# DocF/multispectral-object-detection

Hardware: AMD Instinct MI355X
Metric: image-pairs/sec fwd, yolov5l+CFTx3 640×640 bs64, 1/2/4/8 GPU (higher is better)
Workload: dtype bf16; 1 GPU; cfg3 (yolov5l_fusion_transformerx3_FLIR_aligned) two-stream forward, 640x640, 64 pairs/GPU, BN folded, pre-NMS detections; pairs_per_gpu=64, image_size=640, parallelism=batch-shard x1, hip_graph=True, two_hip_streams=False, forwards_in_flight=3, streams_per_forward_in_flight=1, single_in_flight_streams=2

## Files before the change

multispectral-object-detection_amd/csrc/focus_common.h:

```cpp
#pragma once
#include "cft_common.h"

template <typename IN>
__device__ __forceinline__ void load_pair(const IN* p, float scale, float& a, float& b);
template <>
__device__ __forceinline__ void load_pair<float>(const float* p, float scale, float& a, float& b) {
  const float2 t = *reinterpret_cast<const float2*>(p);
  a = t.x * scale;
  b = t.y * scale;
}
template <>
__device__ __forceinline__ void load_pair<f16_t>(const f16_t* p, float scale, float& a, float& b) {
  const f32x2_t t = __builtin_convertvector(*reinterpret_cast<const f16x2_t*>(p), f32x2_t);
  a = t[0] * scale;
  b = t[1] * scale;
}
template <>
__device__ __forceinline__ void load_pair<unsigned char>(const unsigned char* p, float scale, float& a, float& b) {
  const unsigned short t = *reinterpret_cast<const unsigned short*>(p);
  a = (float)(t & 0xffu) * scale;
  b = (float)(t >> 8) * scale;
}
```

multispectral-object-detection_amd/csrc/focus_conv.hip:

```cpp
#include "cft_common.h"
#include "focus_common.h"

struct FocusConvParams {
  const unsigned char* in;
  long sb, sc, sh;
  float scale;
  const unsigned char* w;
  const float* bias;
  unsigned char* y;
  int kpad, ldy, yoff;
  int Ho, Wo, tiles_x, bands;
};

template <typename T, typename IN, int NT, int ACT>
__global__ void __launch_bounds__(512) focus_conv_kernel(const FocusConvParams p) {
  constexpr int N = NT * 16, TW = 64, TH = 4, PW = TW + 2, PH = TH + 2;
  constexpr int W_BYTES = 3 * N * 128;
  constexpr int ZERO_OFF = PH * PW * 32;
  constexpr int SLD = N + 4;
  constexpr int VPR = N / 8;
  extern __shared__ __attribute__((aligned(16))) unsigned char smem[];
  unsigned char* sW = smem;
  unsigned char* sZ = smem + W_BYTES;

  const int tid = threadIdx.x, lane = tid & 63;
  const int wave = __builtin_amdgcn_readfirstlane(tid >> 6);
  const int lrow = lane & 15, lgrp = lane >> 4;
  const int b = blockIdx.x / p.bands, band = blockIdx.x - b * p.bands;
  const int y0 = band * TH;

  for (int idx = tid; idx < 3 * N * 8; idx += 512) {
    const int kt = idx / (N * 8);
    const int r = idx - kt * (N * 8);
    const int n = r >> 3, s = r & 7, g = s ^ (n & 7);
    *reinterpret_cast<gran_t*>(sW + kt * (N * 128) + n * 128 + (s << 4)) =
        *reinterpret_cast<const gran_t*>(p.w + ((long)n * p.kpad + kt * 64 + g * 8) * 2);
  }
  float bias_v[NT];
#pragma unroll
  for (int j = 0; j < NT; ++j) bias_v[j] = p.bias != nullptr ? p.bias[j * 16 + lrow] : 0.0f;
  float* stage = reinterpret_cast<float*>(sZ) + wave * (16 * SLD);
  const IN* img = reinterpret_cast<const IN*>(p.in) + (long)b * p.sb;
  const int wrow = wave >> 1, wx = (wave & 1) * 32;
  const int y = y0 + wrow;

  const bool owner = tid < PH * PW;
  const int py = tid / PW, px = tid - py * PW;
  const int zy = y0 - 1 + py;
  float raw[12];
#define FOCUS_FETCH(tx_)                                                                            \
  {                                                                                                 \
    const int zx = (tx_) * TW - 1 + px;                                                             \
    _Pragma("unroll") for (int e = 0; e < 12; ++e) raw[e] = 0.0f;                                   \
    if (owner && (unsigned)zy < (unsigned)p.Ho && (unsigned)zx < (unsigned)p.Wo) {                  \
      _Pragma("unroll") for (int c = 0; c < 3; ++c) {                                               \
        const IN* base = img + (long)c * p.sc + (long)(2 * zy) * p.sh + 2 * zx;                     \
        load_pair<IN>(base, p.scale, raw[0 + c], raw[6 + c]);         \
        load_pair<IN>(base + p.sh, p.scale, raw[3 + c], raw[9 + c]);  \
      }                                                                                             \
    }                                                                                               \
  }
  FOCUS_FETCH(0)

  for (int tx = 0; tx < p.tiles_x; ++tx) {
    const int x0 = tx * TW;
    if (owner) {
      float v[16];
#pragma unroll
      for (int e = 0; e < 12; ++e) v[e] = raw[e];
      v[12] = v[13] = v[14] = v[15] = 0.0f;
      gran_t* o = reinterpret_cast<gran_t*>(sZ + tid * 32);
      o[0] = Elem<T>::pack(v);
      o[1] = Elem<T>::pack(v + 8);
    }
    if (tid == PH * PW) *reinterpret_cast<gran_t*>(sZ + ZERO_OFF) = gran_t{0u, 0u, 0u, 0u};
    lds_barrier();
    if (tx + 1 < p.tiles_x) FOCUS_FETCH(tx + 1)

    f32x4_t acc[2][NT];
#pragma unroll
    for (int i = 0; i < 2; ++i)
#pragma unroll
      for (int j = 0; j < NT; ++j) acc[i][j] = f32x4_t{0.f, 0.f, 0.f, 0.f};
#pragma unroll
    for (int ks = 0; ks < 5; ++ks) {
      const int tap = ks * 2 + (lgrp >> 1), half = lgrp & 1;
      const int kh = tap / 3, kw = tap - kh * 3;
      const int abase = tap < 9 ? ((wrow + kh) * PW + wx + lrow + kw) * 32 + half * 16 : ZERO_OFF;
      const int astep = tap < 9 ? 16 * 32 : 0;
      gran_t af[2], bf[NT];
#pragma unroll
      for (int i = 0; i < 2; ++i) af[i] = *reinterpret_cast<const gran_t*>(sZ + abase + i * astep);
      const int kg = (ks & 1) * 4 + lgrp;
#pragma unroll
      for (int j = 0; j < NT; ++j) {
        const int n = j * 16 + lrow;
        bf[j] = *reinterpret_cast<const gran_t*>(sW + (ks >> 1) * (N * 128) + n * 128 + ((kg ^ (n & 7)) << 4));
      }
#pragma unroll
      for (int i = 0; i < 2; ++i)
#pragma unroll
        for (int j = 0; j < NT; ++j) acc[i][j] = mma_granule<T>(af[i], bf[j], acc[i][j]);
    }
    lds_barrier();

#pragma unroll
    for (int i = 0; i < 2; ++i) {
#pragma unroll
      for (int j = 0; j < NT; ++j)
#pragma unroll
        for (int e = 0; e < 4; ++e)
          stage[(lgrp * 4 + e) * SLD + j * 16 + lrow] = apply_act<ACT>(acc[i][j][e] + bias_v[j]);
      __builtin_amdgcn_fence(__ATOMIC_RELEASE, "wavefront");
      __builtin_amdgcn_wave_barrier();
      __builtin_amdgcn_fence(__ATOMIC_ACQUIRE, "wavefront");
      for (int it = lane; it < 16 * VPR; it += 64) {
        const int row = it / VPR, col = (it - row * VPR) * 8;
        const int x = x0 + wx + i * 16 + row;
        if (x < p.Wo && y < p.Ho) {
          const f32x4_t s0 = *reinterpret_cast<const f32x4_t*>(stage + row * SLD + col);
          const f32x4_t s1 = *reinterpret_cast<const f32x4_t*>(stage + row * SLD + col + 4);
          const float v[8] = {s0[0], s0[1], s0[2], s0[3], s1[0], s1[1], s1[2], s1[3]};
          const long m = ((long)b * p.Ho + y) * p.Wo + x;
          *reinterpret_cast<gran_t*>(p.y + (m * p.ldy + p.yoff + col) * 2) = Elem<T>::pack(v);
        }
      }
      __builtin_amdgcn_fence(__ATOMIC_RELEASE, "wavefront");
      __builtin_amdgcn_wave_barrier();
      __builtin_amdgcn_fence(__ATOMIC_ACQUIRE, "wavefront");
    }
    lds_barrier();
  }
#undef FOCUS_FETCH
}

template <typename T, typename IN, int NT, int ACT>
static int launch_focus_conv(const FocusConvParams& p, int B, hipStream_t stream) {
  constexpr int N = NT * 16;
  constexpr int patch = 6 * 66 * 32 + 16, strips = 8 * 16 * (N + 4) * 4;
  constexpr int smem_bytes = 3 * N * 128 + (patch > strips ? patch : strips);
  cft_allow_lds<&focus_conv_kernel<T, IN, NT, ACT>>(smem_bytes);
  hipLaunchKernelGGL((focus_conv_kernel<T, IN, NT, ACT>), dim3(B * p.bands), dim3(512), smem_bytes, stream, p);
  return cft_check_launch("focus_conv_kernel");
}

template <typename T, typename IN, int ACT>
static int dispatch_focus_conv(const FocusConvParams& p, int B, int n, hipStream_t stream) {
  switch (n) {
    case 32: return launch_focus_conv<T, IN, 2, ACT>(p, B, stream);
    case 48: return launch_focus_conv<T, IN, 3, ACT>(p, B, stream);
    case 64: return launch_focus_conv<T, IN, 4, ACT>(p, B, stream);
    default: return launch_focus_conv<T, IN, 5, ACT>(p, B, stream);
  }
}
template <typename T, typename IN>
static int dispatch_focus_act(const FocusConvParams& p, int B, int n, int act, hipStream_t stream) {
  return act == CFT_ACT_SILU ? dispatch_focus_conv<T, IN, CFT_ACT_SILU>(p, B, n, stream) : dispatch_focus_conv<T, IN, CFT_ACT_NONE>(p, B, n, stream);
}
template <typename T>
static int dispatch_focus_in(const FocusConvParams& p, int B, int n, int act, int in_kind, hipStream_t stream) {
  if (in_kind == 1) return dispatch_focus_act<T, unsigned char>(p, B, n, act, stream);
  if constexpr (sizeof(T) == 2 && !__is_same(T, uint16_t)) {
    if (in_kind == 2) return dispatch_focus_act<T, f16_t>(p, B, n, act, stream);
  }
  return dispatch_focus_act<T, float>(p, B, n, act, stream);
}

extern "C" int cft_focus_conv(const void* in, int in_kind, long stride_b, long stride_c, long stride_h, float scale,
                              const void* w, int kpad, const float* bias, void* y, int ldy, int yoff,
                              int B, int H, int W, int n, int act, int dtype, void* stream) {
  CFT_REQUIRE(in && w && y, "cft_focus_conv: null pointer");
  CFT_REQUIRE(dtype == CFT_BF16 || dtype == CFT_F16, "cft_focus_conv: dtype must be CFT_BF16 or CFT_F16");
  CFT_REQUIRE(in_kind >= 0 && in_kind <= 2, "cft_focus_conv: in_kind must be 0 (float), 1 (uint8) or 2 (half)");
  CFT_REQUIRE(in_kind != 2 || dtype == CFT_F16, "cft_focus_conv: half images require dtype CFT_F16");
  CFT_REQUIRE(B > 0 && H > 0 && W > 0 && (H % 2 == 0) && (W % 2 == 0), "cft_focus_conv: H and W must be even");
  CFT_REQUIRE(n == 32 || n == 48 || n == 64 || n == 80, "cft_focus_conv: n must be 32, 48, 64 or 80 (use cft_focus_s2d + cft_conv2d otherwise)");
  CFT_REQUIRE(kpad == 192, "cft_focus_conv: weights must be packed as [n][192] (3x3 taps x 16 channels, zero padded)");
  CFT_REQUIRE(act == CFT_ACT_SILU || act == CFT_ACT_NONE, "cft_focus_conv: activation must be SiLU or none");
  CFT_REQUIRE(ldy % 8 == 0 && yoff % 8 == 0 && ldy >= yoff + n, "cft_focus_conv: bad output ld/offset");
  CFT_REQUIRE(stride_h >= W && stride_c > 0 && stride_b > 0, "cft_focus_conv: bad strides");
  const long es = in_kind == 1 ? 1 : (in_kind == 2 ? 2 : 4);
  CFT_REQUIRE(((long)(size_t)in * 1 % (2 * es) == 0) && stride_h % 2 == 0 && stride_c % 2 == 0 && stride_b % 2 == 0,
              "cft_focus_conv: image rows must start on pixel-pair boundaries (pointer and strides even)");
  FocusConvParams p;
  p.in = (const unsigned char*)in; p.sb = stride_b; p.sc = stride_c; p.sh = stride_h; p.scale = scale;
  p.w = (const unsigned char*)w; p.bias = bias; p.y = (unsigned char*)y;
  p.kpad = kpad; p.ldy = ldy; p.yoff = yoff;
  p.Ho = H / 2; p.Wo = W / 2; p.tiles_x = (p.Wo + 63) / 64; p.bands = (p.Ho + 3) / 4;
  CFT_REQUIRE((long)B * p.bands < (1L << 31) && (long)B * p.Ho * p.Wo * ldy < (1L << 40), "cft_focus_conv: tensor too large");
  hipStream_t s = as_stream(stream);
  return dtype == CFT_BF16 ? dispatch_focus_in<uint16_t>(p, B, n, act, in_kind, s) : dispatch_focus_in<f16_t>(p, B, n, act, in_kind, s);
}
```

Baseline: 3689 image-pairs/sec.

## Separate focus-conv staging LDS from patch to overlap next-tile build with epilogue

When LDS allows, the focus conv kernel now gives the output staging strips their own region, separate from the input patch. This lets the next tile's patch be built and its global fetch issued right after the MMA loop, overlapping the epilogue stores and removing one barrier per tile. Raw image bits are now held undecoded in registers and converted only at build time, which cuts live registers. Weight loads are batched before the LDS stores. In exchange LDS use per block goes up, which may lower occupancy, and the control flow is more complex.

```diff
diff --git a/multispectral-object-detection_amd/csrc/focus_common.h b/multispectral-object-detection_amd/csrc/focus_common.h
--- a/multispectral-object-detection_amd/csrc/focus_common.h
+++ b/multispectral-object-detection_amd/csrc/focus_common.h
@@ -2,22 +2,40 @@
 #include "cft_common.h"
 
 template <typename IN>
-__device__ __forceinline__ void load_pair(const IN* p, float scale, float& a, float& b);
+struct ImagePair;
 template <>
-__device__ __forceinline__ void load_pair<float>(const float* p, float scale, float& a, float& b) {
-  const float2 t = *reinterpret_cast<const float2*>(p);
-  a = t.x * scale;
-  b = t.y * scale;
+struct ImagePair<float> {
+  typedef float2 bits;
+  static __device__ __forceinline__ bits zero() { return float2{0.0f, 0.0f}; }
+  static __device__ __forceinline__ bits load(const float* p) { return *reinterpret_cast<const float2*>(p); }
+  static __device__ __forceinline__ void convert(bits t, float scale, float& a, float& b) {
+    a = t.x * scale;
+    b = t.y * scale;
+  }
+};
+template <>
+struct ImagePair<f16_t> {
+  typedef f16x2_t bits;
+  static __device__ __forceinline__ bits zero() { return f16x2_t{(f16_t)0.0f, (f16_t)0.0f}; }
+  static __device__ __forceinline__ bits load(const f16_t* p) { return *reinterpret_cast<const f16x2_t*>(p); }
+  static __device__ __forceinline__ void convert(bits h, float scale, float& a, float& b) {
+    const f32x2_t t = __builtin_convertvector(h, f32x2_t);
+    a = t[0] * scale;
+    b = t[1] * scale;
+  }
+};
+template <>
+struct ImagePair<unsigned char> {
+  typedef unsigned short bits;
+  static __device__ __forceinline__ bits zero() { return 0; }
+  static __device__ __forceinline__ bits load(const unsigned char* p) { return *reinterpret_cast<const unsigned short*>(p); }
+  static __device__ __forceinline__ void convert(bits t, float scale, float& a, float& b) {
+    a = (float)(t & 0xffu) * scale;
+    b = (float)(t >> 8) * scale;
+  }
+};
+
+template <typename IN>
+__device__ __forceinline__ void load_pair(const IN* p, float scale, float& a, float& b) {
+  ImagePair<IN>::convert(ImagePair<IN>::load(p), scale, a, b);
 }
-template <>
-__device__ __forceinline__ void load_pair<f16_t>(const f16_t* p, float scale, float& a, float& b) {
-  const f32x2_t t = __builtin_convertvector(*reinterpret_cast<const f16x2_t*>(p), f32x2_t);
-  a = t[0] * scale;
-  b = t[1] * scale;
-}
-template <>
-__device__ __forceinline__ void load_pair<unsigned char>(const unsigned char* p, float scale, float& a, float& b) {
-  const unsigned short t = *reinterpret_cast<const unsigned short*>(p);
-  a = (float)(t & 0xffu) * scale;
-  b = (float)(t >> 8) * scale;
-}
diff --git a/multispectral-object-detection_amd/csrc/focus_conv.hip b/multispectral-object-detection_amd/csrc/focus_conv.hip
--- a/multispectral-object-detection_amd/csrc/focus_conv.hip
+++ b/multispectral-object-detection_amd/csrc/focus_conv.hip
@@ -12,6 +12,13 @@
   int Ho, Wo, tiles_x, bands;
 };
 
+template <int N>
+struct focus_lds {
+  static constexpr int weights = 3 * N * 128, patch = 6 * 66 * 32 + 16, strips = 8 * 16 * (N + 4) * 4;
+  static constexpr bool separate = weights + patch + strips <= 80 * 1024;
+  static constexpr int bytes = weights + (separate ? patch + strips : (patch > strips ? patch : strips));
+};
+
 template <typename T, typename IN, int NT, int ACT>
 __global__ void __launch_bounds__(512) focus_conv_kernel(const FocusConvParams p) {
   constexpr int N = NT * 16, TW = 64, TH = 4, PW = TW + 2, PH = TH + 2;
@@ -19,27 +26,41 @@
   constexpr int ZERO_OFF = PH * PW * 32;
   constexpr int SLD = N + 4;
   constexpr int VPR = N / 8;
+  constexpr bool SEP = focus_lds<N>::separate;
   extern __shared__ __attribute__((aligned(16))) unsigned char smem[];
   unsigned char* sW = smem;
   unsigned char* sZ = smem + W_BYTES;
+  unsigned char* sS = SEP ? sZ + focus_lds<N>::patch : sZ;
 
   const int tid = threadIdx.x, lane = tid & 63;
   const int wave = __builtin_amdgcn_readfirstlane(tid >> 6);
   const int lrow = lane & 15, lgrp = lane >> 4;
   const int b = blockIdx.x / p.bands, band = blockIdx.x - b * p.bands;
-  const int y0 = band * TH;
-
-  for (int idx = tid; idx < 3 * N * 8; idx += 512) {
+  const int y0 = band * TH, ntiles = p.tiles_x;
+
+  constexpr int W_PASSES = (3 * N * 8 + 511) / 512;
+  gran_t wv[W_PASSES];
+#pragma unroll
+  for (int i = 0; i < W_PASSES; ++i) {
+    const int idx = tid + i * 512;
     const int kt = idx / (N * 8);
     const int r = idx - kt * (N * 8);
-    const int n = r >> 3, s = r & 7, g = s ^ (n & 7);
-    *reinterpret_cast<gran_t*>(sW + kt * (N * 128) + n * 128 + (s << 4)) =
-        *reinterpret_cast<const gran_t*>(p.w + ((long)n * p.kpad + kt * 64 + g * 8) * 2);
+    const int n = r >> 3, g = (r & 7) ^ (n & 7);
+    if (idx < 3 * N * 8) wv[i] = *reinterpret_cast<const gran_t*>(p.w + ((long)n * p.kpad + kt * 64 + g * 8) * 2);
+  }
+#pragma unroll
+  for (int i = 0; i < W_PASSES; ++i) {
+    const int idx = tid + i * 512;
+    const int kt = idx / (N * 8);
+    const int r = idx - kt * (N * 8);
+    if (idx < 3 * N * 8) *reinterpret_cast<gran_t*>(sW + kt * (N * 128) + (r >> 3) * 128 + ((r & 7) << 4)) = wv[i];
   }
   float bias_v[NT];
 #pragma unroll
   for (int j = 0; j < NT; ++j) bias_v[j] = p.bias != nullptr ? p.bias[j * 16 + lrow] : 0.0f;
-  float* stage = reinterpret_cast<float*>(sZ) + wave * (16 * SLD);
+#pragma unroll
+  for (int j = 0; j < NT; ++j) asm volatile("" : "+v"(bias_v[j]));
+  float* stage = reinterpret_cast<float*>(sS) + wave * (16 * SLD);
   const IN* img = reinterpret_cast<const IN*>(p.in) + (long)b * p.sb;
   const int wrow = wave >> 1, wx = (wave & 1) * 32;
   const int y = y0 + wrow;
@@ -47,35 +68,48 @@
   const bool owner = tid < PH * PW;
   const int py = tid / PW, px = tid - py * PW;
   const int zy = y0 - 1 + py;
-  float raw[12];
-#define FOCUS_FETCH(tx_)                                                                            \
+  typedef ImagePair<IN> Pair;
+  typename Pair::bits raw[6];
+  bool raw_in = false;
+  int f_tx = 0;
+#define FOCUS_FETCH()                                                                               \
   {                                                                                                 \
-    const int zx = (tx_) * TW - 1 + px;                                                             \
-    _Pragma("unroll") for (int e = 0; e < 12; ++e) raw[e] = 0.0f;                                   \
-    if (owner && (unsigned)zy < (unsigned)p.Ho && (unsigned)zx < (unsigned)p.Wo) {                  \
+    const int zx = f_tx * TW - 1 + px;                                                              \
+    raw_in = owner && (unsigned)zy < (unsigned)p.Ho && (unsigned)zx < (unsigned)p.Wo;               \
+    if (raw_in) {                                                                                   \
       _Pragma("unroll") for (int c = 0; c < 3; ++c) {                                               \
         const IN* base = img + (long)c * p.sc + (long)(2 * zy) * p.sh + 2 * zx;                     \
-        load_pair<IN>(base, p.scale, raw[0 + c], raw[6 + c]);         \
-        load_pair<IN>(base + p.sh, p.scale, raw[3 + c], raw[9 + c]);  \
+        raw[c] = Pair::load(base);                                    \
+        raw[3 + c] = Pair::load(base + p.sh);                         \
       }                                                                                             \
     }                                                                                               \
-  }
-  FOCUS_FETCH(0)
-
-  for (int tx = 0; tx < p.tiles_x; ++tx) {
-    const int x0 = tx * TW;
-    if (owner) {
-      float v[16];
-#pragma unroll
-      for (int e = 0; e < 12; ++e) v[e] = raw[e];
-      v[12] = v[13] = v[14] = v[15] = 0.0f;
-      gran_t* o = reinterpret_cast<gran_t*>(sZ + tid * 32);
-      o[0] = Elem<T>::pack(v);
-      o[1] = Elem<T>::pack(v + 8);
-    }
-    if (tid == PH * PW) *reinterpret_cast<gran_t*>(sZ + ZERO_OFF) = gran_t{0u, 0u, 0u, 0u};
+    ++f_tx;                                                                                         \
+  }
+#define FOCUS_BUILD()                                                                               \
+  {                                                                                                 \
+    if (owner) {                                                                                    \
+      float v[16];    \
+      _Pragma("unroll") for (int e = 0; e < 16; ++e) v[e] = 0.0f;                                   \
+      if (raw_in) {                                                                                 \
+        _Pragma("unroll") for (int c = 0; c < 3; ++c) {                                             \
+          Pair::convert(raw[c], p.scale, v[0 + c], v[6 + c]);                                       \
+          Pair::convert(raw[3 + c], p.scale, v[3 + c], v[9 + c]);                                   \
+        }                                                                                           \
+      }                                                                                             \
+      gran_t* o = reinterpret_cast<gran_t*>(sZ + tid * 32);                                         \
+      o[0] = Elem<T>::pack(v);                                                                      \
+      o[1] = Elem<T>::pack(v + 8);                                                                  \
+    }                                                                                               \
+    if (tid == PH * PW) *reinterpret_cast<gran_t*>(sZ + ZERO_OFF) = gran_t{0u, 0u, 0u, 0u};        \
+  }
+  FOCUS_FETCH()
+  FOCUS_BUILD()
+  if (SEP && ntiles > 1) FOCUS_FETCH()
+
+  for (int t = 0; t < ntiles; ++t) {
+    const int x0 = t * TW;
     lds_barrier();
-    if (tx + 1 < p.tiles_x) FOCUS_FETCH(tx + 1)
+    if (!SEP && t + 1 < ntiles) FOCUS_FETCH()
 
     f32x4_t acc[2][NT];
 #pragma unroll
@@ -103,6 +137,10 @@
         for (int j = 0; j < NT; ++j) acc[i][j] = mma_granule<T>(af[i], bf[j], acc[i][j]);
     }
     lds_barrier();
+    if (SEP && t + 1 < ntiles) {
+      FOCUS_BUILD()
+      if (t + 2 < ntiles) FOCUS_FETCH()
+    }
 
 #pragma unroll
     for (int i = 0; i < 2; ++i) {
@@ -129,16 +167,19 @@
       __builtin_amdgcn_wave_barrier();
       __builtin_amdgcn_fence(__ATOMIC_ACQUIRE, "wavefront");
     }
-    lds_barrier();
+    if constexpr (!SEP) {
+      lds_barrier();
+      if (t + 1 < ntiles) FOCUS_BUILD()
+    }
   }
 #undef FOCUS_FETCH
+#undef FOCUS_BUILD
 }
 
 template <typename T, typename IN, int NT, int ACT>
 static int launch_focus_conv(const FocusConvParams& p, int B, hipStream_t stream) {
   constexpr int N = NT * 16;
-  constexpr int patch = 6 * 66 * 32 + 16, strips = 8 * 16 * (N + 4) * 4;
-  constexpr int smem_bytes = 3 * N * 128 + (patch > strips ? patch : strips);
+  constexpr int smem_bytes = focus_lds<N>::bytes;
   cft_allow_lds<&focus_conv_kernel<T, IN, NT, ACT>>(smem_bytes);
   hipLaunchKernelGGL((focus_conv_kernel<T, IN, NT, ACT>), dim3(B * p.bands), dim3(512), smem_bytes, stream, p);
   return cft_check_launch("focus_conv_kernel");
```

Result: no change. 3691 image-pairs/sec, median of 2 (+0.0%).
